# CentaureaHO/CTC-VR

Measured on AMD Instinct MI355X. Metric: audio-frames/sec, streaming RNN-T greedy decode, higher is better.
Workload: dtype bf16x3; 1 GPU; configs[1]: batch=64/GPU synthetic 10 s 80-dim fbank, streaming chunk=16 (online_rnnt_decode.py semantics), greedy decode, whole-utterance call (tokens identical to the per-chunk API); streams_per_gpu=64, chunk_frames=16, chunks=62, weights=seeded synthetic (seed 0, blank_bias 12.0), parallelism=streams sharded x1, no data-path collective

## Files before the change

### ctc-vr_amd/build.py

```python
import os
import subprocess
import sys

HERE = os.path.dirname(os.path.abspath(__file__))
SRC = os.path.join(HERE, "csrc", "rnnt_api.hip")
DEPS = sorted(os.path.join(HERE, "csrc", f) for f in os.listdir(os.path.join(HERE, "csrc"))) + [os.path.join(os.path.dirname(HERE), "include", "rnnt_hip.h")]
LIB = os.path.join(HERE, "librnnt_hip.so")


def lib_path():
    return LIB


def needs_build():
    if not os.path.exists(LIB):
        return True
    t = os.path.getmtime(LIB)
    return any(os.path.getmtime(d) > t for d in DEPS)


def build(force=False, verbose=False):
    if not force and not needs_build():
        return LIB
    hipcc = os.environ.get("HIPCC", "/opt/rocm/bin/hipcc")
    cmd = [hipcc, "-O3", "-std=c++17", "--offload-arch=gfx950", "-fPIC", "-shared", "-Wall", "-Wno-unused-function",
           "-o", LIB, SRC]
    if verbose:
        cmd.insert(1, "-Rpass-analysis=kernel-resource-usage")
        print(" ".join(cmd))
    r = subprocess.run(cmd, capture_output=True, text=True)
    if r.returncode != 0:
        sys.stderr.write(r.stdout + r.stderr)
        raise RuntimeError("hipcc failed building librnnt_hip.so")
    if verbose:
        sys.stderr.write(r.stderr)
    return LIB


if __name__ == "__main__":
    build(force=True, verbose="-v" in sys.argv)
    print(LIB)
```

### ctc-vr_amd/csrc/api_lifecycle.hip.inc

```

int rnnt_abi_version(void) { return 3; }

const char* rnnt_last_error(const rnnt_ctx* ctx) { return ctx ? ctx->err.c_str() : "null context"; }

int rnnt_create(const rnnt_config* cfg, rnnt_ctx** out) {
    if (!cfg || !out) return RNNT_ERR_ARG;
    *out = nullptr;
    rnnt_ctx* ctx = new rnnt_ctx();
    ctx->cfg = *cfg;
    *out = ctx;
    if (cfg->max_streams < 1 || cfg->max_chunk_frames < 7 || cfg->max_cache_frames < 1 || cfg->max_cache_frames > RNNT_PE_LEN ||
        cfg->max_enc_frames < 1 || cfg->max_tokens < 1 || cfg->vocab_size < 2 || cfg->blank_id < 0 || cfg->blank_id >= cfg->vocab_size ||
        cfg->n_steps < 1 || cfg->max_beam < 0 || cfg->max_beam > 64)
        return fail(ctx, RNNT_ERR_ARG, "rnnt_create: bad config");
    HIPCHK(hipSetDevice(cfg->device));
    if (const char* ng = getenv("RNNT_NO_GRAPH")) ctx->use_graphs = (ng[0] == '1') ? 0 : 1;
    if (const char* pe = getenv("RNNT_PERSISTENT")) ctx->use_persistent = (pe[0] == '0') ? 0 : 1;
    if (const char* me = getenv("RNNT_DEC_MULTI")) ctx->use_multi = (me[0] == '0') ? 0 : 1;
    HIPCHK(hipDeviceGetAttribute(&ctx->n_cus, hipDeviceAttributeMultiprocessorCount, cfg->device));
    if (const char* ae = getenv("RNNT_ATTN_STREAM")) ctx->attn_stream = (ae[0] == '0') ? 0 : 1;
    if (const char* be = getenv("RNNT_BEAM_CHAIN")) ctx->use_beam_chain = (be[0] == '0') ? 0 : 1;
    if (const char* fu = getenv("RNNT_FUSED")) ctx->use_fused = atoi(fu);
    if (const char* fe = getenv("RNNT_FUSE_AFTER_NORM")) ctx->fuse_after_norm = (fe[0] == '0') ? 0 : 1;
    if (const char* me = getenv("RNNT_WF_MERGE")) { const int m = atoi(me); ctx->wf_merge = m < 1 ? 1 : (m > WF_MERGE_MAX ? WF_MERGE_MAX : m); }
    if (const char* le = getenv("RNNT_LM")) ctx->use_lm = (le[0] == '0') ? 0 : 1;
    if (const char* ae2 = getenv("RNNT_AS")) ctx->use_as = (ae2[0] == '0') ? 0 : 1;
    if (const char* e_ = getenv("RNNT_LM_PW2_HEAD")) ctx->lm_pw2_head = atoi(e_);
    if (const char* e_ = getenv("RNNT_LM_FFN_MERGE")) ctx->lm_ffn_merge = atoi(e_);
    if (const char* e_ = getenv("RNNT_LM_SIDE")) ctx->lm_side = atoi(e_);
    if (const char* e_ = getenv("RNNT_LM_QKV_TAIL")) ctx->lm_qkv_tail = atoi(e_);
    if (const char* e_ = getenv("RNNT_LM_OUT_CHAIN")) ctx->lm_out_chain = atoi(e_);
    if (const char* e_ = getenv("RNNT_ATTN_BF")) ctx->attn_bf = atoi(e_);
    if (const char* e_ = getenv("RNNT_ATTN_RESIDENT")) ctx->attn_resident = atoi(e_);
    if (const char* e_ = getenv("RNNT_CONV1_FUSE")) ctx->conv1_fuse = atoi(e_);
    if (const char* se = getenv("RNNT_WF_SUB_ASYNC")) ctx->wf_sub_async = (se[0] == '0') ? 0 : 1;
    const int B = cfg->max_streams;
    ctx->tmax = sub_len(cfg->max_chunk_frames);
    ctx->t1max = sub1_len(cfg->max_chunk_frames);
    ctx->cap = RNNT_LORDER + WF_MERGE_MAX * ctx->tmax;
    ctx->tcap = cfg->max_cache_frames;
    ctx->fcap = cfg->max_enc_frames;
    ctx->fstride = ctx->fcap + 1;
    ctx->vpad = (cfg->vocab_size + 31) / 32 * 32;
    const size_t M = (size_t)B * ctx->tmax;
    int rc;
#define ALLOC(p, n) if ((rc = reserve(ctx, ctx->p, (size_t)(n)))) return rc
    ALLOC(y1, (size_t)B * ctx->t1max * RNNT_F1 * D);
    ALLOC(y2, M * RNNT_FSUB * D);
    ALLOC(x, M * D);
    ALLOC(hbuf, M * FF);
    ALLOC(qbuf, M * D);
    ALLOC(abuf, M * D);
    ALLOC(dbuf, M * D);
    ALLOC(kcache, (size_t)L * B * ctx->tcap * D);
    ALLOC(vcache, (size_t)L * B * ctx->tcap * D);
    ALLOC(gring, (size_t)L * B * ctx->cap * D);
    ALLOC(xring, (size_t)L * B * ctx->cap * D);
    ALLOC(encbuf, (size_t)B * ctx->fstride * D);
    ALLOC(encp, (size_t)B * ctx->fstride * D);
    ALLOC(h, (size_t)2 * B * D); ALLOC(c, (size_t)2 * B * D); ALLOC(sel, B); ALLOC(key, B);
    ALLOC(pred, (size_t)B * D); ALLOC(z, (size_t)B * D); ALLOC(logits, (size_t)B * ctx->vpad);
    ALLOC(tok, B); ALLOC(fidx, B); ALLOC(nsym, B); ALLOC(count, B); ALLOC(tokens, (size_t)B * cfg->max_tokens);
    ALLOC(n_active, 4); ALLOC(klen, B); ALLOC(dec_ctrl, 32);
    ALLOC(gm_dbg, 16);
    ALLOC(gm_x1, (size_t)2 * B * GM_PARTS * GM_X1);
    ALLOC(gm_xa, (size_t)2 * B * GM_PARTS * 2 * GREEDY_KF);
    if (cfg->max_beam > 0) {
        ctx->max_rows = B * cfg->max_beam;
        const size_t R = ctx->max_rows, NS = cfg->n_steps, KB = cfg->max_beam;
        ALLOC(pool[0], R * (NS + 1) * 512); ALLOC(pool[1], R * (NS + 1) * 512);
        ALLOC(bpred, R * D); ALLOC(bz, R * D); ALLOC(blogits, R * ctx->vpad);
        ALLOC(b_blank, R * NS); ALLOC(b_toplp, R * NS * KB); ALLOC(b_toptok, R * NS * KB);
        ALLOC(b_tok, R); ALLOC(b_frame, R); ALLOC(b_active, R); ALLOC(b_steps, R); ALLOC(b_srcrow, R); ALLOC(b_srcstep, R);
    }
    ALLOC(scratch, std::max((size_t)L * RNNT_H * ctx->tcap * 128, (size_t)B * ctx->fstride * D));
    ALLOC(pinned, 16);
#undef ALLOC
    HIPCHK(hipMemset(ctx->encbuf, 0, (size_t)B * ctx->fstride * D * sizeof(float)));
    HIPCHK(hipMemset(ctx->encp, 0, (size_t)B * ctx->fstride * D * sizeof(float)));
    return RNNT_OK;
}

void rnnt_destroy(rnnt_ctx* ctx) {
    if (ctx) delete ctx;
}

int64_t rnnt_live_device_bytes(void) { return live_device_bytes.load(); }
// ... 397 lines not shown
```

### ctc-vr_amd/csrc/host_launch.hip.inc

```

namespace {

int fail(rnnt_ctx* ctx, int code, const char* fmt, ...) {
    char buf[512];
    va_list ap;
    va_start(ap, fmt);
    vsnprintf(buf, sizeof(buf), fmt, ap);
    va_end(ap);
    if (ctx) ctx->err = buf;
    return code;
}

#define HIPCHK(expr)                                                                                   \
    do {                                                                                               \
        hipError_t e_ = (expr);                                                                        \
        if (e_ != hipSuccess) return fail(ctx, RNNT_ERR_HIP, "%s failed: %s", #expr, hipGetErrorString(e_)); \
    } while (0)

#define LAUNCHCHK(name)                                                                                \
    do {                                                                                               \
        hipError_t e_ = hipGetLastError();                                                             \
        if (e_ != hipSuccess) return fail(ctx, RNNT_ERR_HIP, "launch %s failed: %s", name, hipGetErrorString(e_)); \
        ctx->launches++;                                                                               \
    } while (0)

enum { TAG_NONE = 0, TAG_CONV1 = 1, TAG_CONV2 = 2, TAG_EMBED = 3, TAG_FFN1 = 4, TAG_FFN2 = 5, TAG_QKV = 6, TAG_ATTN = 7, TAG_ATTN_OUT = 8,
       TAG_PW1 = 9, TAG_DWCONV = 10, TAG_PW2 = 11, TAG_LN = 12, TAG_ENC_PROJ = 13, TAG_LSTM = 20, TAG_PRED_PROJ = 21,
       TAG_JOINT_TANH = 22, TAG_JOINT_OUT = 23, TAG_GREEDY_UPDATE = 24, TAG_BLOCK_FRONT = 30, TAG_BLOCK_BACK = 31, TAG_FFN_FUSED = 32, TAG_FFN_QKV = 33, TAG_OUT_PW1 = 34, TAG_FFN_MERGED = 35,
       TAG_CONV1_MINOR = 36, TAG_CONV2_MINOR = 37, TAG_EMBED_MINOR = 38,
       TAG_SCORE_PICK = 40, TAG_SCORE_ALPHA = 41,
       TAG_SCORE_VITERBI = 42,
       TAG_PREFIX_STEP = 43, TAG_PREFIX_MERGE = 44,
       TAG_CTC_PREFIX = 45,
       TAG_CTC_PREFIX_POOL = 46, TAG_CTC_PREFIX_PACK = 47 };

struct ProfScope {
    rnnt_ctx* ctx; hipStream_t s; bool on;
    ProfScope(rnnt_ctx* c, hipStream_t st, int tag) : ctx(c), s(st), on(c->prof_tag == tag && tag != TAG_NONE && !c->capturing) {
        if (on) {
            if (ctx->prof_used + 2 > ctx->prof_ev.size()) {
                for (int i = 0; i < 2; ++i) { hipEvent_t e; (void)hipEventCreate(&e); ctx->prof_ev.push_back(e); }
            }
            (void)hipEventRecord(ctx->prof_ev[ctx->prof_used], s);
        }
    }
    ~ProfScope() {
        if (on) { (void)hipEventRecord(ctx->prof_ev[ctx->prof_used + 1], s); ctx->prof_used += 2; }
    }
};

template <typename T, bool HOST>
int dmalloc(rnnt_ctx* ctx, DevBuf<T, HOST>& b, size_t n) {
    const size_t bytes = n * sizeof(T);
    void* q = nullptr;
    const hipError_t e = HOST ? hipHostMalloc(&q, bytes) : hipMalloc(&q, bytes);
    if (e != hipSuccess) {
        (void)hipGetLastError();
        return fail(ctx, HOST ? RNNT_ERR_HIP : RNNT_ERR_OOM, "%s of %zu bytes failed", HOST ? "hipHostMalloc" : "hipMalloc", bytes);
    }
    b.p = static_cast<T*>(q);
    b.cap = q ? n : 0;
    if (!HOST) live_device_bytes += (int64_t)(b.cap * sizeof(T));
    return RNNT_OK;
}

template <typename T, bool HOST>
int reserve(rnnt_ctx* ctx, DevBuf<T, HOST>& b, size_t n) {
    if (n <= b.cap) return RNNT_OK;
    b.release();
    return dmalloc(ctx, b, n);
}

template <typename T>
int reserve_exact(rnnt_ctx* ctx, DevBuf<T>& b, size_t n) {
    if (n != b.cap) b.release();
    return reserve(ctx, b, n);
}

template <typename T>
struct Carve {
    T* base = nullptr;
    size_t off = 0;
// ... 245 lines not shown

int run_layer(rnnt_ctx* ctx, hipStream_t s, int l, int B, int tq, int T2, int kv_row0, int pos_start, int ring_pos,
              const int* klen_dev) {
    LayerDescs d;
    LayerBufs bf{ctx->x, ctx->hbuf, ctx->qbuf, ctx->abuf, ctx->dbuf};
    int rc = build_layer(ctx, l, B, tq, T2, kv_row0, pos_start, ring_pos, klen_dev, bf, d);
    if (rc) return rc;
    if ((rc = launch_gemm(ctx, s, &d.ffn1m, 1, TAG_FFN1))) return rc;
    if ((rc = launch_gemm(ctx, s, &d.ffn2m, 1, TAG_FFN2))) return rc;
    if ((rc = launch_gemm(ctx, s, d.qkv, 3, TAG_QKV))) return rc;
    if ((rc = launch_attn(ctx, s, d.attn, B))) return rc;
    if ((rc = launch_gemm(ctx, s, &d.out, 1, TAG_ATTN_OUT))) return rc;
    if ((rc = launch_gemm(ctx, s, &d.pw1, 1, TAG_PW1))) return rc;
    if ((rc = launch_dw(ctx, s, d.dw))) return rc;
    if ((rc = launch_gemm(ctx, s, &d.pw2, 1, TAG_PW2))) return rc;
    if ((rc = launch_gemm(ctx, s, &d.ffn1, 1, TAG_FFN1))) return rc;
    if ((rc = launch_gemm(ctx, s, &d.ffn2, 1, TAG_FFN2))) return rc;
    return launch_ln(ctx, s, d.lnf);
}

static bool conv2_bw_on() {
    static const int conv2_bw = getenv("RNNT_CONV2_BW") ? atoi(getenv("RNNT_CONV2_BW")) : 1;
    return conv2_bw != 0;
}
static bool conv2_fused(const rnnt_ctx* ctx, long long M) {
    return ctx->conv1_fuse && ctx->numerics != RNNT_NUM_F32 && conv2_bw_on() && ctx->conv2_wp && M >= 32768 && M < (1ll << 31);
}
int run_subsample(rnnt_ctx* ctx, hipStream_t s, const float* fbank, int B, int Tstride, int T, const int* starts_dev, int nc,
                  float* y1, float* y2, float* xout, int out_cn = 0, int out_rows = 0, int out_r0 = 0, bool minor = false, bool fuse_ok = false) {
    const int tag1 = minor ? TAG_CONV1_MINOR : TAG_CONV1, tag2 = minor ? TAG_CONV2_MINOR : TAG_CONV2, tag3 = minor ? TAG_EMBED_MINOR : TAG_EMBED;
    const int t1 = sub1_len(T), tq = sub_len(T);
    const int VB = nc * B;
    int rc;
    const bool fused = fuse_ok && conv2_fused(ctx, (long long)VB * tq * RNNT_FSUB);
    if (!fused) {
        if (!y1) return fail(ctx, RNNT_ERR_STATE, "run_subsample: no conv1 slab");
        ProfScope prof(ctx, s, tag1);
        static const int c1_rows = getenv("RNNT_CONV1_ROWS") ? atoi(getenv("RNNT_CONV1_ROWS")) : 1;
        if (c1_rows && !ctx->gemm_m_cap && (long long)VB * ((t1 + C1_TB - 1) / C1_TB) >= 256)
            hipLaunchKernelGGL(conv1_relu_rows, dim3(VB, (t1 + C1_TB - 1) / C1_TB), dim3(256), 0, s, fbank, ctx->conv1_wt, ctx->conv1_b, y1, B, Tstride, t1,
                               starts_dev, nc, out_cn > 0 ? 1 : 0);
        else
            hipLaunchKernelGGL(conv1_relu, dim3(grid_for((long long)VB * t1 * RNNT_F1 * D)), dim3(256), 0, s, fbank, ctx->conv1_wt, ctx->conv1_b,
                               y1, B, Tstride, t1, starts_dev, nc, out_cn > 0 ? 1 : 0);
        LAUNCHCHK("conv1_relu");
    }
    GemmP g = plain_gemm(y1, 0, ctx->conv2_w, 2304, ctx->conv2_b, y2, D, VB * tq * RNNT_FSUB, D, 2304, EPI_RELU);
    g.a_n1 = tq * RNNT_FSUB; g.a_n2 = RNNT_FSUB;
    g.a_s0 = (long long)t1 * RNNT_F1 * D; g.a_s1 = 2LL * RNNT_F1 * D; g.a_s2 = 2LL * D;
    g.a_seg = 768; g.a_seg_stride = (long long)RNNT_F1 * D;
    static const int conv2_lds = getenv("RNNT_CONV2_LDS") ? atoi(getenv("RNNT_CONV2_LDS")) : 1;
    const bool conv2_bw = conv2_bw_on();
    static const bool nw8 = getenv("RNNT_BW_NW") ? atoi(getenv("RNNT_BW_NW")) == 8 : true;
#define BW_LAUNCH_NUM(KERNEL, NUM_, ...) { if (nw8) hipLaunchKernelGGL((KERNEL<NUM_, 8>), grid, dim3(512), 0, s, __VA_ARGS__); \
                                           else hipLaunchKernelGGL((KERNEL<NUM_, 4>), grid, dim3(256), 0, s, __VA_ARGS__); }
#define BW_LAUNCH(KERNEL, ...)                                                                         \
    switch (ctx->numerics) {                                                                           \
        case RNNT_NUM_BF16: BW_LAUNCH_NUM(KERNEL, RNNT_NUM_BF16, __VA_ARGS__) break;                   \
        case RNNT_NUM_F16X3: BW_LAUNCH_NUM(KERNEL, RNNT_NUM_F16X3, __VA_ARGS__) break;                 \
        default: BW_LAUNCH_NUM(KERNEL, RNNT_NUM_BF16X3, __VA_ARGS__) break;                            \
    }                                                                                                  \
    LAUNCHCHK(#KERNEL)
    if (fused) {
        ProfScope prof(ctx, s, tag2);
        g.A = nullptr;
        if ((rc = prepare_gemm(ctx, g))) return rc;
        const dim3 grid((g.M + 127) / 128);
        const Conv1Src src{fbank, ctx->conv1_wt, ctx->conv1_b, starts_dev, B, Tstride, nc, out_cn > 0 ? 1 : 0};
        BW_LAUNCH(gemm_bw_c1, g, ctx->conv2_wp, src);
    } else if (ctx->numerics != RNNT_NUM_F32 && conv2_bw && ctx->conv2_wp && g.M >= 32768 && !ctx->gemm_m_cap) {
        ProfScope prof(ctx, s, tag2);
        if ((rc = prepare_gemm(ctx, g))) return rc;
        const dim3 grid((g.M + 127) / 128);
        BW_LAUNCH(gemm_bw, g, ctx->conv2_wp);
#undef BW_LAUNCH
#undef BW_LAUNCH_NUM
    } else if (ctx->numerics != RNNT_NUM_F32) {
        if ((rc = launch_gemm(ctx, s, &g, 1, tag2))) return rc;
    } else if (conv2_lds && g.M >= 2048 && !ctx->gemm_m_cap) {
        ProfScope prof(ctx, s, tag2);
        GemmBatch gb;
        memset(&gb, 0, sizeof(gb));
        gb.g[0] = g;
        if ((rc = prepare_gemm(ctx, gb.g[0]))) return rc;
        if (conv2_lds == 2 && nc > 1) launch_gemm_ns<2, 2, false, true>(s, gb, g.M, g.N, 1);
        else launch_gemm_ns<2, 2>(s, gb, g.M, g.N, 1);
        LAUNCHCHK("gemm_ns");
    } else if ((rc = launch_gemm(ctx, s, &g, 1, tag2))) return rc;
    GemmP go = plain_gemm(y2, RNNT_FSUB * D, ctx->emb_w, RNNT_FSUB * D, ctx->emb_b, xout, D, VB * tq, D, RNNT_FSUB * D, EPI_SCALE, 16.0f);
    if (out_cn > 0) { go.c_n = out_cn; go.c_s0 = (long long)out_rows * D; go.c_r0 = out_r0; go.c_mod = BIG; go.c_s1 = D; }
    return launch_gemm(ctx, s, &go, 1, tag3);
}

template <int NUM>
size_t fuse_lds(int MT, bool back) {
    const size_t R = 16 * MT, opb = FuseCfg<NUM>::OPB;
    return back ? R * 1024 + R * opb + R * 1024 + sizeof(FuseRows) : R * 1024 + 2 * R * opb + sizeof(FuseRows);
}
template <int NUM, int MT>
int launch_fused_t(rnnt_ctx* ctx, hipStream_t s, bool back, const FuseItem* tab, int n_items, int n_groups, int S, int B) {
    const size_t lds = fuse_lds<NUM>(MT, back);
    int rc_attr;
    const dim3 grid((unsigned)((n_items + 7) / 8 * 8 * n_groups));
    if (back) {
        if ((rc_attr = ensure_dyn_lds(ctx, reinterpret_cast<const void*>(&block_back<NUM, MT>), lds))) return rc_attr;
        hipLaunchKernelGGL((block_back<NUM, MT>), grid, dim3(FUSE_THREADS), lds, s, ctx->layers_dev, tab, ctx->wf_x, n_items, n_groups, S, B, ctx->cap);
        LAUNCHCHK("block_back");
    } else {
        if ((rc_attr = ensure_dyn_lds(ctx, reinterpret_cast<const void*>(&block_front<NUM, MT>), lds))) return rc_attr;
        hipLaunchKernelGGL((block_front<NUM, MT>), grid, dim3(FUSE_THREADS), lds, s, ctx->layers_dev, tab, ctx->wf_x, n_items, n_groups, S, B, (long long)ctx->tcap);
        LAUNCHCHK("block_front");
    }
    return RNNT_OK;
}
template <int NUM>
int launch_fused_n(rnnt_ctx* ctx, hipStream_t s, bool back, const FuseItem* tab, int n_items, int n_groups, int S, int B, int MT) {
    switch (MT) {
        case 1: return launch_fused_t<NUM, 1>(ctx, s, back, tab, n_items, n_groups, S, B);
        case 2: return launch_fused_t<NUM, 2>(ctx, s, back, tab, n_items, n_groups, S, B);
        default: return launch_fused_t<NUM, 3>(ctx, s, back, tab, n_items, n_groups, S, B);
    }
}
int launch_fused(rnnt_ctx* ctx, hipStream_t s, bool back, const FuseItem* tab, int n_items, int maxnf, int B, int tag) {
    ProfScope prof(ctx, s, tag);
// ... 116 lines not shown
```

### ctc-vr_amd/csrc/rnnt_api.hip

```cpp
#include "rnnt_kernels.hip.h"
#include "../../include/rnnt_hip.h"

#include <climits>
#include <cmath>
#include <cstdarg>
#include <cstdio>
#include <chrono>
#include <cstdlib>
#include <cstring>
#include <functional>
#include <map>
#include <string>
#include <algorithm>
#include <array>
#include <atomic>
#include <vector>

namespace {

constexpr int D = RNNT_D, FF = RNNT_FF, L = RNNT_L, DK = RNNT_DK;
constexpr int BIG = INT_MAX;

struct LayerW {
    const float *ln_ffm_g, *ln_ffm_b, *w1m, *b1m, *w2m, *b2m;
// ... 99 lines not shown
    DevBuf<float> encbuf, encp;
    DevBuf<float> h, c, pred, z, logits;
    DevBuf<int> tok, fidx, nsym, count, tokens, n_active, klen, sel;
    DevBuf<unsigned long long> key;
    DevBuf<int> dec_ctrl;
    int use_persistent = 1;
    int attn_stream = 1;
    int fuse_after_norm = 1;
    int overlap_ok = -1;
    int use_multi = 1;
    int n_cus = 0;
    DevBuf<unsigned long long> gm_x1, gm_xa;
    DevBuf<long long> gm_dbg;
    const float *wjc = nullptr, *bjc = nullptr;
    const float *wctc = nullptr, *bctc = nullptr;
    int max_rows = 0;
    DevBuf<float> pool[2], bpred, bz, blogits, b_blank, b_toplp;
    DevBuf<int> b_tok, b_frame, b_active, b_steps, b_toptok, b_srcrow, b_srcstep;
    int pool_cur = 0;
    PinnedBuf<int> pinned;
    DevBuf<float> scratch;

    int n_streams = 0;
    SlotPos pos{0, 0, 0};
    int frames_buffered = 0, frames_decoded = 0;
    int64_t launches = 0, greedy_steps = 0;
    std::vector<SlotPos> slot_pos;
    bool pool_mode = false;
    DevBuf<int> pool_tab;
    PinnedBuf<int> pool_tab_host;
    hipEvent_t pool_ev = nullptr;
    int gemm_m_cap = 0;
    DevBuf<float> wf_x, wf_h, wf_q, wf_a, wf_d, wf_y1, wf_y2;
    int wf_slab = 0;
    DevBuf<int> wf_starts;
    DevBuf<GemmP> wf_gtab; DevBuf<AttnP> wf_atab; DevBuf<DwP> wf_dtab; DevBuf<LnP> wf_ltab;
    hipStream_t dec_stream = nullptr;
    hipStream_t sub_stream = nullptr;
    int wf_sub_async = 1;
    int wf_merge = 2;
    struct WfLaunch { WfType type; int off, n, maxM, maxT2; };
    std::vector<WfLaunch> wf_seq;
    std::vector<std::array<int, 13>> wf_lstart;
    std::vector<int> wf_sc_first, wf_key;
    std::vector<hipEvent_t> ev_pool;
    int use_lm = 1;
    int lm_pw2_head = 2;
    int lm_ffn_merge = 0;
    int lm_qkv_tail = 1, lm_out_chain = 1;
    int lm_side = 1;
    int attn_bf = 1;
    int attn_resident = 1;
    int conv1_fuse = 1;
    DevBuf<float> lm_x, lm_h, lm_q, lm_a, lm_d, lm_g, lm_y1, lm_y2;
    DevBuf<float> lm_y1b, lm_y2b;
    hipEvent_t sub_ev[2] = {nullptr, nullptr};
    DevBuf<float> rg_fb, rg_xt;
    DevBuf<int2> rg_ent;
    DevBuf<LmBlock> lm_blocks;
    std::vector<LmBlock> lm_blocks_host;
    std::vector<int> lm_key;
    DevBuf<LmResHdr> lm_rhdr;
    DevBuf<LmRow> lm_rrows;
    std::vector<LmResHdr> lm_rhdr_host;
    std::vector<LmRow> lm_rrows_host;
    int lm_res_ok = 0, lm_res_stride = 0;
    struct Hyp { std::vector<int> tokens; double log_prob; };
    std::vector<std::vector<Hyp>> beams;
    int use_beam_chain = 1;
    DevBuf<int> bd_tok, bd_len, bd_nh, bd_fend;
    DevBuf<double> bd_sc;
    DevBuf<unsigned long long> bd_hs;
    DevBuf<float> ps_pool[2];
    DevBuf<int> ps_tok, ps_len, ps_nh;
    DevBuf<double> ps_sc;
    DevBuf<unsigned long long> ps_hs;
    std::vector<int> ps_cur, ps_lbound;
    DevBuf<float> fb_dft, fb_mel, fb_pad, fb_spec, fb_pow;
    int fb_rate = 0, fb_nfft = 0;
    DevBuf<float> sc_f, sc_lat;
    DevBuf<int> sc_i;
    DevBuf<double> sc_nll;
    DevBuf<unsigned> al_bp;
    DevBuf<double> al_out;
    DevBuf<float> pb_f;
    DevBuf<int> pb_i;
    DevBuf<double> pb_d, pb_out;
    CtxGraph cg;
    bool cg_on = false;
    DevBuf<int> cg_i, cp_i;
    DevBuf<double> cg_d, cp_d;
    DevBuf<float> cp_lp;
    struct PcSlot { int frames_done, beam, use_context; int64_t gen; };
    std::vector<PcSlot> pc_slot;
    int64_t cg_gen = 0;
    DevBuf<CpSlotState> pc_state;
    DevBuf<int2> pc_parena, pc_tarena;
    DevBuf<int> pc_tab;
    PinnedBuf<int> pc_tab_host;
    hipEvent_t pc_ev = nullptr;
    DevBuf<double> pc_out;
    hipStream_t cap_stream = nullptr;
    struct DecGraph { int n_streams, k; hipGraphExec_t exec; };
    std::vector<DecGraph> dec_graphs;
    bool capturing = false;
    int use_graphs = 1;
// ... 31 lines not shown
```

### ctc-vr_amd/csrc/rnnt_gemm_as.hip.h

```cpp
#pragma once

#ifdef AS_TRACE
__device__ long long as_trace[4096 * 8];
#define AS_STAMP(k_) { if (lane == 0 && blockIdx.x < 1024) as_trace[(blockIdx.x * 4 + wave) * 8 + (k_)] = (long long)__builtin_amdgcn_s_memrealtime(); }
#else
#define AS_STAMP(k_)
#endif
#define AS_MT_ 3
#ifndef BW_WD
#define BW_WD 3
#endif
#ifndef BW_ABL
#define BW_ABL 0
#endif
#ifndef FFN_ABL2
#define FFN_ABL2 0
#endif
struct AsBatch {
    GemmP g[3];
    const uint4* wp[3];
    int ng;
};

template <int MT, int NTW = 4>
// ... 678 lines not shown
        f32x4_ tacc[3][MT][NTW];
        int ug = 0, uh = 0;
#pragma unroll
        for (int u = 0; u < 3; ++u) {
            if (ug >= P.n_tail) break;
            int ng = ug, nh = uh + 1;
            if (nh * 256 >= P.tg[ug].N) { ++ng; nh = 0; }
#pragma unroll
            for (int mt = 0; mt < MT; ++mt)
#pragma unroll
                for (int t = 0; t < NTW; ++t) tacc[u][mt][t] = (f32x4_){0.f, 0.f, 0.f, 0.f};
            const uint4* Wp = P.twp[ug];
            const int ct0 = (uh * NW + wave) * NTW;
#pragma unroll
            for (int ks = 0; ks < 8; ks += 2 * KU) {
                if (u > 0 || ks > 0) tload(b1, Wp, ct0, ks + KU);
                umma(tacc[u], b0, ks, Top);
                if (ks + 2 * KU < 8) tload(b0, Wp, ct0, ks + 2 * KU);
                else if (ng < P.n_tail) tload(b0, P.twp[ng], (nh * NW + wave) * NTW, 0);
                umma(tacc[u], b1, ks + KU, Top);
            }
            ug = ng; uh = nh;
        }
#pragma unroll
        for (int ps = 0; ps < NPS; ++ps) {
            const int row = (tid >> 4) + 4 * NW * ps, m = bm0 + row;
            if (row < R && m < P.M) {
#pragma unroll
                for (int j = 0; j < 4; ++j) stg4(P.Y + (long long)m * RNNT_D + 4 * ((tid & 15) + 16 * j), ykeep[ps][j]);
            }
        }
        ug = 0; uh = 0;
#pragma unroll
        for (int u = 0; u < 3; ++u) {
            if (ug >= P.n_tail) break;
            as_epilogue_t<MT, NTW>(P.tg[ug], tacc[u], bm0, (uh * NW + wave) * CW, lane);
            if (++uh * 256 >= P.tg[ug].N) { ++ug; uh = 0; }
        }
    }
}

struct Conv1Src {
    const float* x;
    const float* w1t;
    const float* b1;
    const int* starts;
    int B, T, n_chunks, b_major;
};
#if defined(__HIP_DEVICE_COMPILE__)
__device__ __forceinline__ float ldc1(const float* p) { return *(const __attribute__((address_space(4))) float*)p; }
#else
__device__ __forceinline__ float ldc1(const float* p) { return *p; }
#endif
template <int NUM, int NW, bool FUSE>
__device__ __forceinline__ void gemm_bw_body(const GemmP& p, const uint4* __restrict__ wp, const Conv1Src& c1) {
    using C = FuseCfg<NUM>;
    constexpr bool F16 = C::F16, LO = C::PLANES == 2;
    constexpr int U = C::PLANES, MT = 8, NTW = 16 / NW, NT = 64 * NW, AJ = NT >= 512 ? 1 : 512 / NT;
    static_assert(!FUSE || NW <= 8, "fused staging maps waves 0..7");
    __shared__ uint4 Ah[2][512];
    __shared__ uint4 Al[LO ? 2 : 1][LO ? 512 : 1];
    const int tid = threadIdx.x, lane = tid & 63, wave = tid >> 6;
    const int i = lane & 15, q = lane >> 4;
    const int bm0 = blockIdx.x * 128;
    if (bm0 >= p.M) return;
    const int uwave = __builtin_amdgcn_readfirstlane(wave);
    const int srow = FUSE ? (uwave >> 2) * 64 + lane : (tid & 511) >> 2, sc = FUSE ? (uwave & 3) : (tid & 3);
    const bool stager = NT <= 512 || tid < 512;
    const float* ag[AJ];
#pragma unroll
    for (int j = 0; j < AJ; ++j) {
        const int m = min(bm0 + srow + (NT / 4) * j, p.M - 1);
        if constexpr (FUSE) {
            const int v = fastdiv(m, p.a_n1, p.a_n1_magic, p.a_n1_shift), r1 = m - v * p.a_n1;
            const int tp = fastdiv(r1, p.a_n2, p.a_n2_magic, p.a_n2_shift), fp = r1 - tp * p.a_n2;
            const int cidx = c1.b_major ? v % c1.n_chunks : v / c1.B, b = c1.b_major ? v / c1.n_chunks : v - cidx * c1.B;
            const int st0 = c1.starts ? ldgi(c1.starts + cidx) : 0;
            ag[j] = c1.x + ((long long)b * c1.T + st0 + 4 * tp) * RNNT_IDIM + 4 * fp;
        } else ag[j] = p.A + a_row_off(p, m);
    }
    const bool aplain = p.a_plain != 0;
    const int KT = p.K >> 5;
    float4 ra[FUSE ? 1 : 4][AJ][2];
    auto gload = [&](float4 (&r)[AJ][2], int blk) {
        if (BW_ABL & 1) { for (int j = 0; j < AJ; ++j) { r[j][0] = make_float4(0.5f, 0.25f, 1.f, 2.f); r[j][1] = r[j][0]; } return; }
        if (!stager) return;
        const int kk = blk * 32 + 8 * sc;
        const long long ko = aplain ? (long long)kk : a_k_off(p, kk);
#pragma unroll
        for (int j = 0; j < AJ; ++j) { r[j][0] = ldg4_nt(ag[j] + ko); r[j][1] = ldg4_nt(ag[j] + ko + 4); }
    };
    float xp[FUSE ? AJ : 1][9], cw[2][FUSE ? 9 : 1][4], cb[2][4];
    auto pload = [&](int tap) {
        const int kh = tap / 3, kw = tap - 3 * kh;
#pragma unroll
        for (int j = 0; j < AJ; ++j)
#pragma unroll
            for (int r = 0; r < 3; ++r)
#pragma unroll
                for (int c = 0; c < 3; ++c) xp[j][r * 3 + c] = ldg1(ag[j] + (2 * kh + r) * RNNT_IDIM + 2 * kw + c);
    };
    auto wload = [&](int blk, int half) {
        const int c0 = (blk & 7) * 32 + 8 * sc + 4 * half;
#pragma unroll
        for (int t = 0; t < 9; ++t)
#pragma unroll
            for (int e = 0; e < 4; ++e) cw[half][t][e] = ldc1(c1.w1t + t * RNNT_D + c0 + e);
#pragma unroll
        for (int e = 0; e < 4; ++e) cb[half][e] = ldc1(c1.b1 + c0 + e);
    };
    auto produce = [&](float4 (&r)[AJ][2], int blk) {
        if (BW_ABL & 1) { for (int j = 0; j < AJ; ++j) { r[j][0] = make_float4(0.5f, 0.25f, 1.f, 2.f); r[j][1] = r[j][0]; } return; }
        wload(blk, 1);
#pragma unroll
        for (int half = 0; half < 2; ++half)
#pragma unroll
            for (int j = 0; j < AJ; ++j) {
                float y[4];
#pragma unroll
                for (int e = 0; e < 4; ++e) {
                    float acc = cb[half][e];
#pragma unroll
                    for (int t = 0; t < 9; ++t) acc = fmaf(xp[j][t], cw[half][t][e], acc);
                    y[e] = fmaxf(acc, 0.f);
                }
                r[j][half] = make_float4(y[0], y[1], y[2], y[3]);
            }
    };
    auto lstore = [&](int buf, const float4 (&r)[AJ][2]) {
        if (!stager) return;
#pragma unroll
        for (int j = 0; j < AJ; ++j) {
            const int rr = srow + (NT / 4) * j;
            uint4 h, l;
            split8_16<F16, LO>(r[j][0], r[j][1], h, l);
            const int slot = rr * 4 + (sc ^ bf_swz(rr));
            Ah[buf][slot] = h;
            if constexpr (LO) Al[buf][slot] = l;
        }
    };
    auto bload = [&](uint4 (&b)[NTW * U], int kt) {
        if (BW_ABL & 2) { for (int t = 0; t < NTW * U; ++t) b[t] = make_uint4(0x3c003c00u + lane, 0x3c003c00u, 0x3c003c00u, 0x3c003c00u); return; }
#pragma unroll
        for (int t = 0; t < NTW; ++t)
#pragma unroll
            for (int u = 0; u < U; ++u) {
#if defined(__HIP_DEVICE_COMPILE__)
                typedef unsigned u32x4g_ __attribute__((ext_vector_type(4)));
                const u32x4g_ v = *(const RNNT_GAS u32x4g_*)(wp + ((long long)((wave * NTW + t) * KT + kt) * U + u) * 64 + lane);
                b[t * U + u] = make_uint4(v[0], v[1], v[2], v[3]);
#else
                b[t * U + u] = wp[((long long)((wave * NTW + t) * KT + kt) * U + u) * 64 + lane];
#endif
            }
    };
    f32x4_ acc[MT][NTW];
#pragma unroll
    for (int mt = 0; mt < MT; ++mt)
#pragma unroll
        for (int t = 0; t < NTW; ++t) acc[mt][t] = (f32x4_){0.f, 0.f, 0.f, 0.f};
    const int fsw = q ^ bf_swz(i);
    auto mma = [&](int buf, const uint4 (&b)[NTW * U]) {
        if (BW_ABL & 4) { for (int t = 0; t < NTW * U; ++t) asm volatile("" :: "v"(b[t].x), "v"(b[t].y), "v"(b[t].z), "v"(b[t].w)); return; }
#pragma unroll
        for (int mt = 0; mt < MT; ++mt) {
            const int slot = (16 * mt + i) * 4 + fsw;
            const uint4 ah = Ah[buf][slot];
            uint4 al = ah;
            if constexpr (LO) al = Al[buf][slot];
#pragma unroll
            for (int t = 0; t < NTW; ++t) {
                if constexpr (LO) {
                    acc[mt][t] = mfma16_<F16>(b[t * U], al, acc[mt][t]);
                    acc[mt][t] = mfma16_<F16>(b[t * U + 1], ah, acc[mt][t]);
                }
                acc[mt][t] = mfma16_<F16>(b[t * U], ah, acc[mt][t]);
            }
        }
    };
    uint4 wb[4][NTW * U];
    if constexpr (FUSE) { pload(0); wload(0, 0); }
    else {
#pragma unroll
        for (int k = 0; k < 4; ++k) gload(ra[k], k);
    }
#pragma unroll
    for (int k = 0; k < BW_WD; ++k) bload(wb[k], k);
    if constexpr (FUSE) produce(ra[0], 0);
    lstore(0, ra[0]);
    __syncthreads();
#ifdef AS_TRACE
    long long bw_t[4] = {0, 0, 0, 0}, bw_last = __builtin_amdgcn_s_memtime();
#define BW_STAMP(k_) { const long long t_ = __builtin_amdgcn_s_memtime(); __builtin_amdgcn_s_waitcnt(0xC07F); bw_t[k_] += t_ - bw_last; bw_last = t_; }
#else
#define BW_STAMP(k_)
#endif
    for (int blk = 0; blk < KT; blk += 4) {
#pragma unroll
        for (int s = 0; s < 4; ++s) {
            const int k = blk + s;
            if (k + BW_WD < KT) bload(wb[(s + BW_WD) & 3], k + BW_WD);
            if constexpr (FUSE) {
                if (k + 1 < KT) { if (((k + 1) & 7) == 0) pload((k + 1) >> 3); wload(k + 1, 0); }
            } else if (k + 4 < KT) gload(ra[s], k + 4);
            BW_STAMP(0)
            mma(s & 1, wb[s]);
            BW_STAMP(1)
            if (k + 1 < KT && !(BW_ABL & 8)) {
                if constexpr (FUSE) { produce(ra[0], k + 1); lstore((s + 1) & 1, ra[0]); }
                else lstore((s + 1) & 1, ra[(s + 1) & 3]);
            }
            BW_STAMP(2)
            if (!(BW_ABL & 16)) __syncthreads();
            BW_STAMP(3)
        }
    }
#ifdef AS_TRACE
    if (lane == 0 && blockIdx.x < 1024 && wave < 4) for (int k_ = 0; k_ < 4; ++k_) as_trace[(blockIdx.x * 4 + wave) * 8 + k_] = bw_t[k_];
#endif
    as_epilogue_t<MT, NTW>(p, acc, bm0, wave * 16 * NTW, lane);
}
template <int NUM, int NW = 4>
__global__ __launch_bounds__(64 * NW) void gemm_bw(GemmP p, const uint4* __restrict__ wp) { gemm_bw_body<NUM, NW, false>(p, wp, Conv1Src{}); }
template <int NUM, int NW = 8>
__global__ __launch_bounds__(64 * NW) void gemm_bw_c1(GemmP p, const uint4* __restrict__ wp, Conv1Src c1) { gemm_bw_body<NUM, NW, true>(p, wp, c1); }
```

Before: 13.07 million audio-frames/s.

## Add two-workgroups-per-CU conv2 GEMM variant with reduced register pipeline depth

Adds gemm_bw_w2 and gemm_bw_c1_w2 variants, enabled by default, that cut the weight run-ahead to one k-step and the A-prefetch depth. They spill fused conv1 patch state and the A pointer to LDS and use buffer loads for weights. The mma loop software-prefetches the next LDS A fragment so the kernel fits in 128 VGPRs and two 512-thread workgroups can share a CU. The build now always emits resource-usage remarks and fails if these kernels spill or exceed 128 VGPRs. The trade is less latency hiding per workgroup in exchange for more resident waves, plus extra LDS traffic.

```diff
diff --git a/ctc-vr_amd/build.py b/ctc-vr_amd/build.py
--- a/ctc-vr_amd/build.py
+++ b/ctc-vr_amd/build.py
@@ -1,4 +1,5 @@
 import os
+import re
 import subprocess
 import sys
 
@@ -19,19 +20,41 @@
     return any(os.path.getmtime(d) > t for d in DEPS)
 
 
+def check_two_per_cu(remarks):
+    found, name = {}, None
+    for line in remarks.splitlines():
+        m = re.search(r"remark: +(Function Name|VGPRs|ScratchSize \[bytes/lane\]|Occupancy \[waves/SIMD\]): (\S+)", line)
+        if not m:
+            continue
+        if m.group(1) == "Function Name":
+            name = m.group(2) if re.match(r"_Z\d+gemm_bw(_c1)?_w2", m.group(2)) else None
+            if name:
+                found[name] = {}
+        elif name:
+            found[name][m.group(1).split()[0]] = int(m.group(2))
+    bad = {k: v for k, v in found.items() if v.get("ScratchSize", 0) != 0 or v.get("Occupancy", 4) < 4 or v.get("VGPRs", 0) > 128}
+    if bad:
+        raise RuntimeError(f"conv2 two-workgroups-per-CU kernels no longer fit 128 VGPRs without scratch: {bad}")
+    return {k: (v.get("VGPRs"), v.get("ScratchSize"), v.get("Occupancy")) for k, v in found.items()}
+
+
 def build(force=False, verbose=False):
     if not force and not needs_build():
         return LIB
     hipcc = os.environ.get("HIPCC", "/opt/rocm/bin/hipcc")
-    cmd = [hipcc, "-O3", "-std=c++17", "--offload-arch=gfx950", "-fPIC", "-shared", "-Wall", "-Wno-unused-function",
+    cmd = [hipcc, "-Rpass-analysis=kernel-resource-usage", "-O3", "-std=c++17", "--offload-arch=gfx950", "-fPIC", "-shared", "-Wall", "-Wno-unused-function",
            "-o", LIB, SRC]
     if verbose:
-        cmd.insert(1, "-Rpass-analysis=kernel-resource-usage")
         print(" ".join(cmd))
     r = subprocess.run(cmd, capture_output=True, text=True)
     if r.returncode != 0:
         sys.stderr.write(r.stdout + r.stderr)
         raise RuntimeError("hipcc failed building librnnt_hip.so")
+    try:
+        check_two_per_cu(r.stderr)
+    except RuntimeError:
+        os.remove(LIB)
+        raise
     if verbose:
         sys.stderr.write(r.stderr)
     return LIB
diff --git a/ctc-vr_amd/csrc/api_lifecycle.hip.inc b/ctc-vr_amd/csrc/api_lifecycle.hip.inc
--- a/ctc-vr_amd/csrc/api_lifecycle.hip.inc
+++ b/ctc-vr_amd/csrc/api_lifecycle.hip.inc
@@ -33,6 +33,7 @@
     if (const char* e_ = getenv("RNNT_ATTN_BF")) ctx->attn_bf = atoi(e_);
     if (const char* e_ = getenv("RNNT_ATTN_RESIDENT")) ctx->attn_resident = atoi(e_);
     if (const char* e_ = getenv("RNNT_CONV1_FUSE")) ctx->conv1_fuse = atoi(e_);
+    if (const char* e_ = getenv("RNNT_BW_WG2")) ctx->bw_wg2 = atoi(e_);
     if (const char* se = getenv("RNNT_WF_SUB_ASYNC")) ctx->wf_sub_async = (se[0] == '0') ? 0 : 1;
     const int B = cfg->max_streams;
     ctx->tmax = sub_len(cfg->max_chunk_frames);
diff --git a/ctc-vr_amd/csrc/host_launch.hip.inc b/ctc-vr_amd/csrc/host_launch.hip.inc
--- a/ctc-vr_amd/csrc/host_launch.hip.inc
+++ b/ctc-vr_amd/csrc/host_launch.hip.inc
@@ -28,6 +28,7 @@
        TAG_PW1 = 9, TAG_DWCONV = 10, TAG_PW2 = 11, TAG_LN = 12, TAG_ENC_PROJ = 13, TAG_LSTM = 20, TAG_PRED_PROJ = 21,
        TAG_JOINT_TANH = 22, TAG_JOINT_OUT = 23, TAG_GREEDY_UPDATE = 24, TAG_BLOCK_FRONT = 30, TAG_BLOCK_BACK = 31, TAG_FFN_FUSED = 32, TAG_FFN_QKV = 33, TAG_OUT_PW1 = 34, TAG_FFN_MERGED = 35,
        TAG_CONV1_MINOR = 36, TAG_CONV2_MINOR = 37, TAG_EMBED_MINOR = 38,
+       TAG_CONV2_WG2 = 39,
        TAG_SCORE_PICK = 40, TAG_SCORE_ALPHA = 41,
        TAG_SCORE_VITERBI = 42,
        TAG_PREFIX_STEP = 43, TAG_PREFIX_MERGE = 44,
@@ -379,7 +380,10 @@
     static const int conv2_lds = getenv("RNNT_CONV2_LDS") ? atoi(getenv("RNNT_CONV2_LDS")) : 1;
     const bool conv2_bw = conv2_bw_on();
     static const bool nw8 = getenv("RNNT_BW_NW") ? atoi(getenv("RNNT_BW_NW")) == 8 : true;
-#define BW_LAUNCH_NUM(KERNEL, NUM_, ...) { if (nw8) hipLaunchKernelGGL((KERNEL<NUM_, 8>), grid, dim3(512), 0, s, __VA_ARGS__); \
+    const bool wg2 = nw8 && ctx->bw_wg2;
+    if (wg2 && g.a_seg % 32 != 0) return fail(ctx, RNNT_ERR_STATE, "run_subsample: gemm_bw_w2 needs whole k-steps inside one A segment");
+#define BW_LAUNCH_NUM(KERNEL, NUM_, ...) { if (wg2) hipLaunchKernelGGL((KERNEL##_w2<NUM_>), grid, dim3(512), 0, s, __VA_ARGS__); \
+                                           else if (nw8) hipLaunchKernelGGL((KERNEL<NUM_, 8>), grid, dim3(512), 0, s, __VA_ARGS__); \
                                            else hipLaunchKernelGGL((KERNEL<NUM_, 4>), grid, dim3(256), 0, s, __VA_ARGS__); }
 #define BW_LAUNCH(KERNEL, ...)                                                                         \
     switch (ctx->numerics) {                                                                           \
@@ -389,14 +393,14 @@
     }                                                                                                  \
     LAUNCHCHK(#KERNEL)
     if (fused) {
-        ProfScope prof(ctx, s, tag2);
+        ProfScope prof(ctx, s, tag2), prof2(ctx, s, wg2 ? TAG_CONV2_WG2 : TAG_NONE);
         g.A = nullptr;
         if ((rc = prepare_gemm(ctx, g))) return rc;
         const dim3 grid((g.M + 127) / 128);
         const Conv1Src src{fbank, ctx->conv1_wt, ctx->conv1_b, starts_dev, B, Tstride, nc, out_cn > 0 ? 1 : 0};
         BW_LAUNCH(gemm_bw_c1, g, ctx->conv2_wp, src);
     } else if (ctx->numerics != RNNT_NUM_F32 && conv2_bw && ctx->conv2_wp && g.M >= 32768 && !ctx->gemm_m_cap) {
-        ProfScope prof(ctx, s, tag2);
+        ProfScope prof(ctx, s, tag2), prof2(ctx, s, wg2 ? TAG_CONV2_WG2 : TAG_NONE);
         if ((rc = prepare_gemm(ctx, g))) return rc;
         const dim3 grid((g.M + 127) / 128);
         BW_LAUNCH(gemm_bw, g, ctx->conv2_wp);
diff --git a/ctc-vr_amd/csrc/rnnt_api.hip b/ctc-vr_amd/csrc/rnnt_api.hip
--- a/ctc-vr_amd/csrc/rnnt_api.hip
+++ b/ctc-vr_amd/csrc/rnnt_api.hip
@@ -175,6 +175,7 @@
     int attn_bf = 1;
     int attn_resident = 1;
     int conv1_fuse = 1;
+    int bw_wg2 = 1;
     DevBuf<float> lm_x, lm_h, lm_q, lm_a, lm_d, lm_g, lm_y1, lm_y2;
     DevBuf<float> lm_y1b, lm_y2b;
     hipEvent_t sub_ev[2] = {nullptr, nullptr};
diff --git a/ctc-vr_amd/csrc/rnnt_gemm_as.hip.h b/ctc-vr_amd/csrc/rnnt_gemm_as.hip.h
--- a/ctc-vr_amd/csrc/rnnt_gemm_as.hip.h
+++ b/ctc-vr_amd/csrc/rnnt_gemm_as.hip.h
@@ -754,14 +754,16 @@
 #else
 __device__ __forceinline__ float ldc1(const float* p) { return *p; }
 #endif
-template <int NUM, int NW, bool FUSE>
+template <int NUM, int NW, bool FUSE, int WA = BW_WD>
 __device__ __forceinline__ void gemm_bw_body(const GemmP& p, const uint4* __restrict__ wp, const Conv1Src& c1) {
     using C = FuseCfg<NUM>;
     constexpr bool F16 = C::F16, LO = C::PLANES == 2;
     constexpr int U = C::PLANES, MT = 8, NTW = 16 / NW, NT = 64 * NW, AJ = NT >= 512 ? 1 : 512 / NT;
     static_assert(!FUSE || NW <= 8, "fused staging maps waves 0..7");
-    __shared__ uint4 Ah[2][512];
-    __shared__ uint4 Al[LO ? 2 : 1][LO ? 512 : 1];
+    static_assert(WA >= 1 && WA <= 3, "weight run-ahead of 1..3 k-steps");
+    constexpr int WR = WA == 1 ? 2 : 4, AR = FUSE ? 1 : WA == 1 ? 1 : 4;
+    __shared__ uint4 Ahl[LO ? 4 : 2][512];
+    uint4 (*const Ah)[512] = Ahl, (*const Al)[512] = Ahl + (LO ? 2 : 0);
     const int tid = threadIdx.x, lane = tid & 63, wave = tid >> 6;
     const int i = lane & 15, q = lane >> 4;
     const int bm0 = blockIdx.x * 128;
@@ -783,24 +785,41 @@
     }
     const bool aplain = p.a_plain != 0;
     const int KT = p.K >> 5;
-    float4 ra[FUSE ? 1 : 4][AJ][2];
+    float4 ra[AR][AJ][2];
     auto gload = [&](float4 (&r)[AJ][2], int blk) {
         if (BW_ABL & 1) { for (int j = 0; j < AJ; ++j) { r[j][0] = make_float4(0.5f, 0.25f, 1.f, 2.f); r[j][1] = r[j][0]; } return; }
         if (!stager) return;
         const int kk = blk * 32 + 8 * sc;
-        const long long ko = aplain ? (long long)kk : a_k_off(p, kk);
+        const long long ko = aplain ? (long long)kk : WA == 1 ? a_k_off(p, blk * 32) + 8 * sc : a_k_off(p, kk);
 #pragma unroll
         for (int j = 0; j < AJ; ++j) { r[j][0] = ldg4_nt(ag[j] + ko); r[j][1] = ldg4_nt(ag[j] + ko + 4); }
     };
     float xp[FUSE ? AJ : 1][9], cw[2][FUSE ? 9 : 1][4], cb[2][4];
-    auto pload = [&](int tap) {
+    auto pload = [&](float (&x)[FUSE ? AJ : 1][9], int tap) {
         const int kh = tap / 3, kw = tap - 3 * kh;
 #pragma unroll
         for (int j = 0; j < AJ; ++j)
 #pragma unroll
             for (int r = 0; r < 3; ++r)
 #pragma unroll
-                for (int c = 0; c < 3; ++c) xp[j][r * 3 + c] = ldg1(ag[j] + (2 * kh + r) * RNNT_IDIM + 2 * kw + c);
+                for (int c = 0; c < 3; ++c) x[j][r * 3 + c] = ldg1(ag[j] + (2 * kh + r) * RNNT_IDIM + 2 * kw + c);
+    };
+    constexpr bool XL = FUSE && WA == 1;
+    __shared__ float xpl[XL ? 11 : 1][XL ? NT : 1];
+    auto agstore = [&]() {
+        const unsigned long long a = (unsigned long long)ag[0];
+        xpl[9][tid] = __uint_as_float((unsigned)a); xpl[10][tid] = __uint_as_float((unsigned)(a >> 32));
+    };
+    auto agload = [&]() {
+        ag[0] = (const float*)((unsigned long long)__float_as_uint(xpl[9][tid]) | (unsigned long long)__float_as_uint(xpl[10][tid]) << 32);
+    };
+    auto xstore = [&](const float (&x)[FUSE ? AJ : 1][9]) {
+#pragma unroll
+        for (int t = 0; t < 9; ++t) xpl[t][tid] = x[0][t];
+    };
+    auto xload = [&]() {
+#pragma unroll
+        for (int t = 0; t < 9; ++t) xp[0][t] = xpl[t][tid];
     };
     auto wload = [&](int blk, int half) {
         const int c0 = (blk & 7) * 32 + 8 * sc + 4 * half;
@@ -849,8 +868,14 @@
             for (int u = 0; u < U; ++u) {
 #if defined(__HIP_DEVICE_COMPILE__)
                 typedef unsigned u32x4g_ __attribute__((ext_vector_type(4)));
-                const u32x4g_ v = *(const RNNT_GAS u32x4g_*)(wp + ((long long)((wave * NTW + t) * KT + kt) * U + u) * 64 + lane);
-                b[t * U + u] = make_uint4(v[0], v[1], v[2], v[3]);
+                if constexpr (WA == 1) {
+                    const auto wrs = __builtin_amdgcn_make_buffer_rsrc(const_cast<uint4*>(wp), 0, 256 * p.K * 2 * U, 0x00020000);
+                    const auto v = __builtin_amdgcn_raw_buffer_load_b128(wrs, 16 * lane, (((uwave * NTW + t) * KT + kt) * U + u) * 1024, 0);
+                    b[t * U + u] = make_uint4(v[0], v[1], v[2], v[3]);
+                } else {
+                    const u32x4g_ v = *(const RNNT_GAS u32x4g_*)(wp + ((long long)((wave * NTW + t) * KT + kt) * U + u) * 64 + lane);
+                    b[t * U + u] = make_uint4(v[0], v[1], v[2], v[3]);
+                }
 #else
                 b[t * U + u] = wp[((long long)((wave * NTW + t) * KT + kt) * U + u) * 64 + lane];
 #endif
@@ -864,6 +889,31 @@
     const int fsw = q ^ bf_swz(i);
     auto mma = [&](int buf, const uint4 (&b)[NTW * U]) {
         if (BW_ABL & 4) { for (int t = 0; t < NTW * U; ++t) asm volatile("" :: "v"(b[t].x), "v"(b[t].y), "v"(b[t].z), "v"(b[t].w)); return; }
+        if constexpr (WA == 1) {
+            constexpr bool LOOK = FUSE;
+            uint4 ah = Ah[buf][i * 4 + fsw], al = ah;
+            if constexpr (LO) al = Al[buf][i * 4 + fsw];
+#pragma unroll
+            for (int mt = 0; mt < MT; ++mt) {
+                const int nslot = (16 * (mt + 1) + i) * 4 + fsw;
+                uint4 nh = ah, nl = al;
+                if (LOOK && mt + 1 < MT) nh = Ah[buf][nslot];
+                if constexpr (LO) {
+#pragma unroll
+                    for (int t = 0; t < NTW; ++t) acc[mt][t] = mfma16_<F16>(b[t * U], al, acc[mt][t]);
+                    __builtin_amdgcn_sched_barrier(0);
+                    if (mt + 1 < MT) nl = Al[buf][nslot];
+#pragma unroll
+                    for (int t = 0; t < NTW; ++t) acc[mt][t] = mfma16_<F16>(b[t * U + 1], ah, acc[mt][t]);
+                }
+#pragma unroll
+                for (int t = 0; t < NTW; ++t) acc[mt][t] = mfma16_<F16>(b[t * U], ah, acc[mt][t]);
+                __builtin_amdgcn_sched_barrier(0);
+                if (!LOOK && mt + 1 < MT) nh = Ah[buf][nslot];
+                ah = nh; al = nl;
+            }
+            return;
+        }
 #pragma unroll
         for (int mt = 0; mt < MT; ++mt) {
             const int slot = (16 * mt + i) * 4 + fsw;
@@ -880,37 +930,52 @@
             }
         }
     };
-    uint4 wb[4][NTW * U];
-    if constexpr (FUSE) { pload(0); wload(0, 0); }
+    uint4 wb[WR][NTW * U];
+    if constexpr (FUSE) { pload(xp, 0); wload(0, 0); if constexpr (XL) { xstore(xp); agstore(); } }
     else {
 #pragma unroll
-        for (int k = 0; k < 4; ++k) gload(ra[k], k);
-    }
-#pragma unroll
-    for (int k = 0; k < BW_WD; ++k) bload(wb[k], k);
+        for (int k = 0; k < AR; ++k) gload(ra[k], k);
+    }
+#pragma unroll
+    for (int k = 0; k < WA; ++k) bload(wb[k], k);
     if constexpr (FUSE) produce(ra[0], 0);
     lstore(0, ra[0]);
     __syncthreads();
 #ifdef AS_TRACE
     long long bw_t[4] = {0, 0, 0, 0}, bw_last = __builtin_amdgcn_s_memtime();
+#ifdef AS_TRACE_SEG
+#define BW_STAMP(k_) { if ((k_) == AS_TRACE_SEG || (k_) == (AS_TRACE_SEG + 3) % 4) { const long long t_ = __builtin_amdgcn_s_memtime(); __builtin_amdgcn_s_waitcnt(0xC07F); \
+                                                                                    if ((k_) == AS_TRACE_SEG) bw_t[k_] += t_ - bw_last; else bw_last = t_; } }
+#else
 #define BW_STAMP(k_) { const long long t_ = __builtin_amdgcn_s_memtime(); __builtin_amdgcn_s_waitcnt(0xC07F); bw_t[k_] += t_ - bw_last; bw_last = t_; }
+#endif
 #else
 #define BW_STAMP(k_)
 #endif
-    for (int blk = 0; blk < KT; blk += 4) {
-#pragma unroll
-        for (int s = 0; s < 4; ++s) {
+    constexpr int UF = WA == 1 ? 2 : 4;
+    for (int blk = 0; blk < KT; blk += UF) {
+#pragma unroll
+        for (int s = 0; s < UF; ++s) {
             const int k = blk + s;
-            if (k + BW_WD < KT) bload(wb[(s + BW_WD) & 3], k + BW_WD);
+            if (k + WA < KT) bload(wb[(s + WA) % WR], k + WA);
             if constexpr (FUSE) {
-                if (k + 1 < KT) { if (((k + 1) & 7) == 0) pload((k + 1) >> 3); wload(k + 1, 0); }
-            } else if (k + 4 < KT) gload(ra[s], k + 4);
+                if (k + 1 < KT) { if (!XL && ((k + 1) & 7) == 0) pload(xp, (k + 1) >> 3); wload(k + 1, 0); }
+            } else if (k + AR < KT) gload(ra[s % AR], k + AR);
             BW_STAMP(0)
-            mma(s & 1, wb[s]);
+            mma(s & 1, wb[s % WR]);
             BW_STAMP(1)
             if (k + 1 < KT && !(BW_ABL & 8)) {
-                if constexpr (FUSE) { produce(ra[0], k + 1); lstore((s + 1) & 1, ra[0]); }
-                else lstore((s + 1) & 1, ra[(s + 1) & 3]);
+                if constexpr (XL) {
+                    static_assert(!XL || AJ == 1, "one row per stager");
+                    float xn[FUSE ? AJ : 1][9];
+                    const bool nt = ((k + 2) & 7) == 0 && k + 2 < KT;
+                    xload();
+                    if (nt) { agload(); pload(xn, (k + 2) >> 3); }
+                    produce(ra[0], k + 1);
+                    lstore((s + 1) & 1, ra[0]);
+                    if (nt) xstore(xn);
+                } else if constexpr (FUSE) { produce(ra[0], k + 1); lstore((s + 1) & 1, ra[0]); }
+                else lstore((s + 1) & 1, ra[(s + 1) % AR]);
             }
             BW_STAMP(2)
             if (!(BW_ABL & 16)) __syncthreads();
@@ -920,9 +985,19 @@
 #ifdef AS_TRACE
     if (lane == 0 && blockIdx.x < 1024 && wave < 4) for (int k_ = 0; k_ < 4; ++k_) as_trace[(blockIdx.x * 4 + wave) * 8 + k_] = bw_t[k_];
 #endif
-    as_epilogue_t<MT, NTW>(p, acc, bm0, wave * 16 * NTW, lane);
+    if constexpr (WA == 1) {
+        int te = threadIdx.x;
+#if defined(__HIP_DEVICE_COMPILE__)
+        asm volatile("" : "+v"(te));
+#endif
+        as_epilogue_t<MT, NTW>(p, acc, bm0, (te >> 6) * 16 * NTW, te & 63);
+    } else as_epilogue_t<MT, NTW>(p, acc, bm0, wave * 16 * NTW, lane);
 }
 template <int NUM, int NW = 4>
 __global__ __launch_bounds__(64 * NW) void gemm_bw(GemmP p, const uint4* __restrict__ wp) { gemm_bw_body<NUM, NW, false>(p, wp, Conv1Src{}); }
 template <int NUM, int NW = 8>
 __global__ __launch_bounds__(64 * NW) void gemm_bw_c1(GemmP p, const uint4* __restrict__ wp, Conv1Src c1) { gemm_bw_body<NUM, NW, true>(p, wp, c1); }
+template <int NUM>
+__global__ __launch_bounds__(512, 4) void gemm_bw_w2(GemmP p, const uint4* __restrict__ wp) { gemm_bw_body<NUM, 8, false, 1>(p, wp, Conv1Src{}); }
+template <int NUM>
+__global__ __launch_bounds__(512, 4) void gemm_bw_c1_w2(GemmP p, const uint4* __restrict__ wp, Conv1Src c1) { gemm_bw_body<NUM, 8, true, 1>(p, wp, c1); }
```

Result: no change. 12.99 million audio-frames/s, median of 2 (-0.6%).
